# ubisoft/ubisoft-laforge-msmd

Hardware: AMD Instinct MI355X
Metric: FLAME frames/sec on 4s@16kHz clips (whole job; MSMD.forward motion-coefficient frames) (higher is better)
Workload: dtype bf16; 1 GPU; configs[1]: MSMD.forward, batch=32 x 4 s clips per GPU, wav2vec2-base encoder + 8-layer motion decoder, eval-mode, synthetic closed-form weights; batch_per_gpu=32, frames_per_clip=100, parallelism=dp1 (independent clips, no collective), launch=one hipGraph replay per step (the batch sits in the captured input buffers)

## Files before the change

### include/msmd_hip.h

```cpp
#ifndef MSMD_HIP_H
#define MSMD_HIP_H

#include <stdint.h>

#ifdef __cplusplus
extern "C" {
#endif

#define MSMD_F32 0
#define MSMD_BF16 1
#define MSMD_F16 2
#define MSMD_F16X2 3

#define MSMD_ACT_NONE 0
#define MSMD_ACT_GELU 1
#define MSMD_ACT_ELU 2

typedef void* msmd_stream_t;

int msmd_abi_version(void);
#define MSMD_GEMM_VARIANT(v) ((v) << 8)
#define MSMD_GEMM_WRITE_THROUGH (1 << 16)
#define MSMD_GEMM_PAIRED_STORES (1 << 17)
#define MSMD_GEMM_STAGGER (1 << 18)
// ... 42 lines not shown
                       const float* gamma, const float* beta, void* y, int rows, int cols, float eps, int dtype,
                       msmd_stream_t stream);

int msmd_layernorm_f16x2(const float* x, const float* residual, const float* gamma, const float* beta,
                         const float* post_add, float* y, void* y_split, int rows, int cols, float eps, int act,
                         msmd_stream_t stream);

int msmd_split_f16x2(const float* x, void* y, long rows, int cols, long ldx, int cols_out, msmd_stream_t stream);
int msmd_unsplit_f16x2(const void* x, float* y, long rows, int cols, int cols_in, long ldy, msmd_stream_t stream);

int msmd_attention_prefetch(const void* Q, const void* K, const void* V, void* O, int B, int H, int Tq, int Tk,
                            long q_bstride, long q_tstride, long k_bstride, long k_tstride, long v_bstride,
                            long v_tstride, long o_bstride, long o_tstride, float scale, const uint8_t* mask, int dtype,
                            const void* const* prefetch_ptrs, const long* prefetch_bytes, int n_prefetch,
                            msmd_stream_t stream);
int msmd_attention(const void* Q, const void* K, const void* V, void* O, int B, int H, int Tq, int Tk,
                   long q_bstride, long q_tstride, long k_bstride, long k_tstride, long v_bstride,
                   long v_tstride, long o_bstride, long o_tstride, float scale, const uint8_t* mask,
                   int dtype, msmd_stream_t stream);

int msmd_attention_f16x2(const void* Q, const void* K, const void* V, void* O, int B, int H, int Tq, int Tk,
                         long q_bstride, long q_tstride, long k_bstride, long k_tstride, long v_bstride,
                         long v_tstride, long o_bstride, long o_tstride, float scale, const uint8_t* mask,
                         int out_dtype, msmd_stream_t stream);


int msmd_person_query_attention(const void* x, long x_seq_stride, const void* Wq, const float* bq, const void* K,
                                const void* V, long kv_bstride, long kv_tstride, void* out, int N, int H, int Tk, int d,
                                float scale, int dtype, msmd_stream_t stream);
int msmd_person_query_attention_ln(const void* x, long x_seq_stride, const void* Wq, const float* bq,
                                   const float* wq_colsum, float ln_eps, const void* K, const void* V, long kv_bstride,
                                   long kv_tstride, void* out, int N, int H, int Tk, int d, float scale, int dtype,
                                   msmd_stream_t stream);

int msmd_attention_dropout(const void* Q, const void* K, const void* V, void* O, int B, int H, int Tq, int Tk,
                           long q_bstride, long q_tstride, long k_bstride, long k_tstride, long v_bstride,
                           long v_tstride, long o_bstride, long o_tstride, float scale, const uint8_t* mask,
                           float p_drop, const unsigned long* rng_state, unsigned int site, int dtype,
                           msmd_stream_t stream);
int msmd_attention_dropout_prefetch(const void* Q, const void* K, const void* V, void* O, int B, int H, int Tq, int Tk,
                                    long q_bstride, long q_tstride, long k_bstride, long k_tstride, long v_bstride,
                                    long v_tstride, long o_bstride, long o_tstride, float scale, const uint8_t* mask,
                                    float p_drop, const unsigned long* rng_state, unsigned int site, int dtype,
                                    const void* const* prefetch_ptrs, const long* prefetch_bytes, int n_prefetch,
                                    msmd_stream_t stream);

int msmd_dropout(const void* x, const void* residual, void* y, long n, float p, const unsigned long* rng_state,
                 unsigned int site, int dtype, msmd_stream_t stream);

int msmd_attention_bwd(const void* Q, const void* K, const void* V, const void* dO, void* dQ, void* dK, void* dV,
                       int B, int H, int Tq, int Tk, long q_bstride, long q_tstride, long k_bstride,
                       long k_tstride, long v_bstride, long v_tstride, long do_bstride, long do_tstride,
                       long dq_bstride, long dq_tstride, long dk_bstride, long dk_tstride, long dv_bstride,
                       long dv_tstride, float scale, const uint8_t* mask, float p_drop,
                       const unsigned long* rng_state, unsigned int site, msmd_stream_t stream);

int msmd_pad_audio(const float* audio, float* out, int B, int L, int reflect_len, int replicate_len,
                   msmd_stream_t stream);

#define MSMD_CONV0_SPLITS 16
int msmd_conv0_stats(const float* audio, const float* w0, float* stats, float* ws, int B, int L, int reflect_len,
                     int replicate_len, int C, float eps, msmd_stream_t stream);

int msmd_conv0_gn_gelu(const float* audio, const float* w0, const float* stats, const float* gamma,
                       const float* beta, void* out, int B, int L, int reflect_len, int replicate_len,
                       int C, int out_dtype, msmd_stream_t stream);
// ... 148 lines not shown
```

### ubisoft-laforge-msmd_amd/csrc/attention.hip

```cpp
#include "common.h"

struct AttnArgs {
  const void* Q; const void* K; const void* V; void* O;
  int B, H, Tq, Tk;
  long qb, qt, kb, kt, vb, vt, ob, ot;
  float scale;
  const uint8_t* mask;
  float p_drop;
  const unsigned long* rng_state;
  unsigned site;
  const void* pf_ptr[4] = {nullptr, nullptr, nullptr, nullptr};
  long pf_bytes[4] = {0, 0, 0, 0};
};

typedef short s16x4 __attribute__((ext_vector_type(4)));

template <typename T, int NW>
__global__ __launch_bounds__(64 * NW) void attn_kernel(const AttnArgs p) {
  constexpr bool BF = sizeof(T) == 2;
  constexpr int KROW = BF ? 128 : 256;
  constexpr int VROW = BF ? 128 : 272;
  constexpr int NCH = BF ? 8 : 16;
  __shared__ __attribute__((aligned(16))) unsigned char smem[64 * KROW + 64 * VROW + 1024];
  unsigned char* sK = smem;
// ... 193 lines not shown
      }
    } else {
#pragma unroll
      for (int f = 0; f < 4; ++f)
#pragma unroll
        for (int e = 0; e < 4; ++e) {
          const int krow = 16 * f + 4 * fq + e;
#pragma unroll
          for (int d = 0; d < 4; ++d) {
            const float a = *(const float*)(sV + krow * 272 + (16 * d + fr) * 4);
            acc_o[d] = __builtin_amdgcn_mfma_f32_16x16x4f32(a, s[f][e], acc_o[d], 0, 0, 0);
          }
        }
    }
  }

  if (query < p.Tq) {
    const float inv = 1.0f / (l_run * (1.0f - p.p_drop));
    T* Op = (T*)p.O + (long)b * p.ob + (long)query * p.ot + h * 64;
#pragma unroll
    for (int d = 0; d < 4; ++d) {
      float o[4];
#pragma unroll
      for (int e = 0; e < 4; ++e) o[e] = acc_o[d][e] * inv;
      if constexpr (BF)
        *(typename Vec4T<T>::type*)(Op + 16 * d + 4 * fq) = pack4<T>(o[0], o[1], o[2], o[3]);
      else
        *(f32x4*)(Op + 16 * d + 4 * fq) = f32x4{o[0], o[1], o[2], o[3]};
    }
  }
}

constexpr int ATTN_WHOLE_NF = 13;

template <typename T, int NW, int NF = ATTN_WHOLE_NF>
__global__ __launch_bounds__(64 * NW) void attn_whole_kernel(const AttnArgs p) {
  static_assert(sizeof(T) == 2, "16-bit storage modes");
  constexpr int ROWS = 16 * NF, NT = 64 * NW;
  extern __shared__ __attribute__((aligned(16))) unsigned char smem[];
  unsigned char* sK = smem;
  const int tid = threadIdx.x, lane = tid & 63, wid = tid >> 6;
  const int fr = lane & 15, fq = lane >> 4;
  const int b = blockIdx.z, h = blockIdx.y;
  const int query = blockIdx.x * (16 * NW) + wid * 16 + fr;
  const int qrow = query < p.Tq ? query : p.Tq - 1;
  const T* Qp = (const T*)p.Q + (long)b * p.qb + (long)qrow * p.qt + h * 64;
  const T* Kb = (const T*)p.K + (long)b * p.kb + h * 64;
  const T* Vb = (const T*)p.V + (long)b * p.vb + h * 64;
  const int nf = (p.Tk + 15) >> 4;
  const int rows = min(((nf + 1) & ~1) * 16, ROWS);
  unsigned char* sV = smem + rows * 128;

  constexpr int NPF = (ROWS * 8 + NT - 1) / NT;
  u32x4 pk[NPF], pv[NPF];
#pragma unroll
  for (int i = 0; i < NPF; ++i) {
    const int c = tid + i * NT, row = min(c >> 3, p.Tk - 1), ch = c & 7;
    pk[i] = *(const u32x4*)(Kb + (long)row * p.kt + ch * 8);
    pv[i] = *(const u32x4*)(Vb + (long)row * p.vt + ch * 8);
  }
  u32x4 qf[2];
#pragma unroll
  for (int g = 0; g < 2; ++g) qf[g] = *(const u32x4*)(Qp + 32 * g + 8 * fq);
  __builtin_amdgcn_sched_barrier(0);
#pragma unroll
  for (int i = 0; i < NPF; ++i) {
    const int c = tid + i * NT, row = c >> 3, ch = c & 7;
    if (row < rows) {
      const bool live = row < p.Tk;
      *(u32x4*)(sK + row * 128 + ((ch ^ ((row >> 1) & 7)) << 4)) = live ? pk[i] : u32x4{0, 0, 0, 0};
      *(u32x4*)(sV + row * 128 + ((((ch >> 1) ^ ((row >> 1) & 3)) << 5) + ((ch & 1) << 4))) = live ? pv[i] : u32x4{0, 0, 0, 0};
    }
  }
  __syncthreads();
  asm volatile("" ::"v"(qf[0]), "v"(qf[1]));
  if (p.pf_bytes[0] > 0) {
    typedef __attribute__((address_space(3))) void lds_sink_t;
    const unsigned sink_lds = (unsigned)(uintptr_t)(lds_sink_t*)smem + 2 * rows * 128;
    unsigned m0_keep;
    const long stride = (long)gridDim.x * gridDim.y * gridDim.z * NT * 16;
    const long wave0 = ((((long)blockIdx.z * gridDim.y + blockIdx.y) * gridDim.x + blockIdx.x) * NT + (tid & ~63)) * 16;
#pragma unroll
    for (int r = 0; r < 4; ++r) {
      const char* base = (const char*)p.pf_ptr[r];
      const long nb = p.pf_bytes[r] & ~1023L;
      for (long off = wave0; off < nb; off += stride)
        asm volatile("s_mov_b32 %0, m0\n\ts_mov_b32 m0, %2\n\ts_nop 0\n\tglobal_load_lds_dwordx4 %1, off\n\ts_mov_b32 m0, %0"
                     : "=&s"(m0_keep) : "v"(base + off + lane * 16), "s"(sink_lds) : "memory");
    }
  }

  f32x4 s[NF];
#pragma unroll
  for (int f = 0; f < NF; ++f) {
    s[f] = f32x4{0.f, 0.f, 0.f, 0.f};
    if (f >= nf) continue;
    const int row = 16 * f + fr;
#pragma unroll
    for (int g = 0; g < 2; ++g) {
      const u32x4 a = *(const u32x4*)(sK + row * 128 + (((4 * g + fq) ^ ((row >> 1) & 7)) << 4));
      s[f] = mfma16<T>(a, qf[g], s[f]);
    }
  }
  if ((p.Tk & 15) || p.mask) {
    const uint8_t* mrow = p.mask ? p.mask + (long)qrow * p.Tk : nullptr;
#pragma unroll
    for (int f = 0; f < NF; ++f) {
      if (f >= nf || !(p.mask || f == nf - 1)) continue;
      const int k0 = 16 * f + 4 * fq;
      unsigned m4 = 0;
      if (mrow) {
        if (k0 + 4 <= p.Tk) __builtin_memcpy(&m4, mrow + k0, 4);
        else {
#pragma unroll
          for (int e = 0; e < 4; ++e)
            if (k0 + e < p.Tk) m4 |= (unsigned)(mrow[k0 + e] != 0) << (8 * e);
        }
      }
#pragma unroll
      for (int e = 0; e < 4; ++e)
        if (k0 + e >= p.Tk || ((m4 >> (8 * e)) & 0xff)) s[f][e] = -INFINITY;
    }
  }
  const float c = p.scale * 1.4426950408889634f;
  float mx = -INFINITY;
#pragma unroll
  for (int f = 0; f < NF; ++f) {
    if (f >= nf) continue;
#pragma unroll
    for (int e = 0; e < 4; ++e) mx = fmaxf(mx, s[f][e]);
  }
  mx = fmaxf(mx, __shfl_xor(mx, 16, 64));
  mx = fmaxf(mx, __shfl_xor(mx, 32, 64));
  const float mc = (mx == -INFINITY) ? 0.f : mx * c;
  float ps = 0.f;
#pragma unroll
  for (int f = 0; f < NF; ++f) {
    if (f >= nf) continue;
#pragma unroll
    for (int e = 0; e < 4; ++e) {
      const float pe = __builtin_amdgcn_exp2f(fmaf(s[f][e], c, -mc));
      s[f][e] = pe;
      ps += pe;
    }
  }
  ps += __shfl_xor(ps, 16, 64);
  ps += __shfl_xor(ps, 32, 64);
  if (p.p_drop > 0.f) {
    const unsigned thr = dropout_threshold16(p.p_drop);
    const unsigned long rowbase = ((unsigned long)(b * p.H + h) * p.Tq + qrow) * 128ul;
#pragma unroll
    for (int pr = 0; pr < (NF + 1) / 2; ++pr) {
      if (2 * pr >= nf) continue;
      const Philox4 r = dropout_bits(p.rng_state, p.site, rowbase + (unsigned long)(4 * pr + fq));
#pragma unroll
      for (int o = 0; o < 2; ++o) {
        if (2 * pr + o >= NF) continue;
#pragma unroll
        for (int e = 0; e < 4; ++e) s[2 * pr + o][e] = dropout_value16(r, e, o) >= thr ? s[2 * pr + o][e] : 0.f;
      }
    }
  }

  f32x4 acc_o[4];
#pragma unroll
  for (int d = 0; d < 4; ++d) acc_o[d] = f32x4{0.f, 0.f, 0.f, 0.f};
  typedef typename Vec8T<T>::type V8;
  typedef short s16x8 __attribute__((ext_vector_type(8)));
  const int qp = fr >> 2, pp = fr & 3;
#pragma unroll
  for (int pr = 0; pr < (NF + 1) / 2; ++pr) {
    const int f0 = 2 * pr, f1 = 2 * pr + 1;
    if (f0 >= nf) continue;
    const f32x4 s1 = f1 < NF ? s[f1 < NF ? f1 : 0] : f32x4{0.f, 0.f, 0.f, 0.f};
    const V8 pbv = V8{(T)s[f0][0], (T)s[f0][1], (T)s[f0][2], (T)s[f0][3], (T)s1[0], (T)s1[1], (T)s1[2], (T)s1[3]};
    const u32x4 pb = __builtin_bit_cast(u32x4, pbv);
    const int r0 = 16 * f0 + 4 * fq + qp, r1 = f1 < NF ? r0 + 16 : r0;
#pragma unroll
    for (int d = 0; d < 4; ++d) {
      const s16x4 v0 = __builtin_amdgcn_ds_read_tr16_b64_v4i16(
          (s16x4 __attribute__((address_space(3)))*)(sV + r0 * 128 + ((d ^ ((r0 >> 1) & 3)) << 5) + pp * 8));
      const s16x4 v1 = __builtin_amdgcn_ds_read_tr16_b64_v4i16(
          (s16x4 __attribute__((address_space(3)))*)(sV + r1 * 128 + ((d ^ ((r1 >> 1) & 3)) << 5) + pp * 8));
      const s16x8 va = s16x8{v0[0], v0[1], v0[2], v0[3], v1[0], v1[1], v1[2], v1[3]};
      acc_o[d] = mfma16<T>(__builtin_bit_cast(u32x4, va), pb, acc_o[d]);
    }
  }
  if (query < p.Tq) {
    const float inv = 1.0f / (ps * (1.0f - p.p_drop));
    T* Op = (T*)p.O + (long)b * p.ob + (long)query * p.ot + h * 64;
#pragma unroll
    for (int d = 0; d < 4; ++d)
      *(typename Vec4T<T>::type*)(Op + 16 * d + 4 * fq) = pack4<T>(acc_o[d][0] * inv, acc_o[d][1] * inv, acc_o[d][2] * inv, acc_o[d][3] * inv);
  }
  asm volatile("s_waitcnt vmcnt(0)" ::: "memory");
}

__device__ __forceinline__ int vsw(int row) { return ((row & 3) << 2) | ((row >> 2) & 3); }

template <typename TO, int NW>
__global__ __launch_bounds__(64 * NW) void attn_split_kernel(const AttnArgs p) {
  __shared__ __attribute__((aligned(16))) unsigned char smem[2 * 64 * 256];
  unsigned char* sK = smem;
  unsigned char* sV = smem + 64 * 256;
  const int tid = threadIdx.x, lane = tid & 63, wid = tid >> 6;
  const int fr = lane & 15, fq = lane >> 4;
  const int b = blockIdx.z, h = blockIdx.y;
  constexpr int NT = 64 * NW;
  const int query = blockIdx.x * (16 * NW) + wid * 16 + fr;
  const int qrow = query < p.Tq ? query : p.Tq - 1;
  const f16_t* Qp = (const f16_t*)p.Q + 2 * ((long)b * p.qb + (long)qrow * p.qt) + h * 128;
  const f16_t* Kb = (const f16_t*)p.K + 2 * (long)b * p.kb + h * 128;
  const f16_t* Vb = (const f16_t*)p.V + 2 * (long)b * p.vb + h * 128;

  u32x4 qh[2], ql[2];
#pragma unroll
  for (int g = 0; g < 2; ++g) {
    qh[g] = *(const u32x4*)(Qp + 64 * g + 8 * fq);
    ql[g] = *(const u32x4*)(Qp + 64 * g + 32 + 8 * fq);
  }
  f32x4 o0[4], o1[4];
#pragma unroll
  for (int d = 0; d < 4; ++d) o0[d] = o1[d] = f32x4{0.f, 0.f, 0.f, 0.f};
  float m_run = -INFINITY, l_run = 0.f;

  constexpr int NPF = (64 * 16 + NT - 1) / NT;
  u32x4 pk[NPF], pv[NPF];
// ... 220 lines not shown
                        o_bstride, o_tstride, scale, mask, 0.f, nullptr, 0u, dtype, stream);
}

extern "C" int msmd_attention_prefetch(const void* Q, const void* K, const void* V, void* O, int B, int H, int Tq, int Tk,
                                       long q_bstride, long q_tstride, long k_bstride, long k_tstride, long v_bstride,
                                       long v_tstride, long o_bstride, long o_tstride, float scale, const uint8_t* mask,
                                       int dtype, const void* const* prefetch_ptrs, const long* prefetch_bytes,
                                       int n_prefetch, msmd_stream_t stream) {
  return attention_impl(Q, K, V, O, B, H, Tq, Tk, q_bstride, q_tstride, k_bstride, k_tstride, v_bstride, v_tstride,
                        o_bstride, o_tstride, scale, mask, 0.f, nullptr, 0u, dtype, stream, prefetch_ptrs, prefetch_bytes,
                        n_prefetch);
}

extern "C" int msmd_attention_dropout(const void* Q, const void* K, const void* V, void* O, int B, int H, int Tq,
                                      int Tk, long q_bstride, long q_tstride, long k_bstride, long k_tstride,
                                      long v_bstride, long v_tstride, long o_bstride, long o_tstride, float scale,
                                      const uint8_t* mask, float p_drop, const unsigned long* rng_state,
                                      unsigned int site, int dtype, msmd_stream_t stream) {
  return attention_impl(Q, K, V, O, B, H, Tq, Tk, q_bstride, q_tstride, k_bstride, k_tstride, v_bstride, v_tstride,
                        o_bstride, o_tstride, scale, mask, p_drop, rng_state, site, dtype, stream);
}

extern "C" int msmd_attention_dropout_prefetch(const void* Q, const void* K, const void* V, void* O, int B, int H, int Tq,
                                               int Tk, long q_bstride, long q_tstride, long k_bstride, long k_tstride,
                                               long v_bstride, long v_tstride, long o_bstride, long o_tstride, float scale,
                                               const uint8_t* mask, float p_drop, const unsigned long* rng_state,
                                               unsigned int site, int dtype, const void* const* prefetch_ptrs,
                                               const long* prefetch_bytes, int n_prefetch, msmd_stream_t stream) {
  return attention_impl(Q, K, V, O, B, H, Tq, Tk, q_bstride, q_tstride, k_bstride, k_tstride, v_bstride, v_tstride,
                        o_bstride, o_tstride, scale, mask, p_drop, rng_state, site, dtype, stream, prefetch_ptrs,
                        prefetch_bytes, n_prefetch);
}

extern "C" int msmd_attention_f16x2(const void* Q, const void* K, const void* V, void* O, int B, int H, int Tq, int Tk,
                                    long q_bstride, long q_tstride, long k_bstride, long k_tstride, long v_bstride,
                                    long v_tstride, long o_bstride, long o_tstride, float scale, const uint8_t* mask,
                                    int out_dtype, msmd_stream_t stream) {
  if (B <= 0 || H <= 0 || Tq <= 0 || Tk <= 0 || !Q || !K || !V || !O) return 1;
  if (out_dtype != MSMD_F32 && out_dtype != MSMD_F16X2) return 1;
  if (q_tstride % 32 || k_tstride % 32 || v_tstride % 32 || q_bstride % 32 || k_bstride % 32 || v_bstride % 32) return 1;
  if (out_dtype == MSMD_F16X2 ? (o_tstride % 32 || o_bstride % 32) : (o_tstride % 4 || o_bstride % 4)) return 1;
  if (((uintptr_t)Q & 15) || ((uintptr_t)K & 15) || ((uintptr_t)V & 15) || ((uintptr_t)O & 15)) return 1;
  AttnArgs p{Q, K, V, O, B, H, Tq, Tk, q_bstride, q_tstride, k_bstride, k_tstride, v_bstride, v_tstride,
             o_bstride, o_tstride, scale, mask, 0.f, nullptr, 0u};
  const int nw = attn_waves(Tq, H, B);
  dim3 grid((Tq + 16 * nw - 1) / (16 * nw), H, B), block(64 * nw);
  hipStream_t st = (hipStream_t)stream;
#define MSMD_ATTN_S(TO)                                                                                \
  do {                                                                                                 \
    if (nw == 4) hipLaunchKernelGGL((attn_split_kernel<TO, 4>), grid, block, 0, st, p);                \
    else if (nw == 7) hipLaunchKernelGGL((attn_split_kernel<TO, 7>), grid, block, 0, st, p);           \
    else if (nw == 13) hipLaunchKernelGGL((attn_split_kernel<TO, 13>), grid, block, 0, st, p);         \
    else hipLaunchKernelGGL((attn_split_kernel<TO, 16>), grid, block, 0, st, p);                       \
  } while (0)
  if (out_dtype == MSMD_F32) MSMD_ATTN_S(float);
  else MSMD_ATTN_S(f16_t);
#undef MSMD_ATTN_S
  MSMD_RETURN_LAST();
}



template <typename T> __device__ __forceinline__ void load8(const T* p, float (&o)[8]) {
  if constexpr (sizeof(T) == 4) {
    const f32x4 a = *(const f32x4*)p, b = *(const f32x4*)(p + 4);
#pragma unroll
// ... 212 lines not shown
```

### ubisoft-laforge-msmd_amd/model.py

```python
from __future__ import annotations

from types import SimpleNamespace

import torch
import torch.nn as nn

from . import init, ops, shapes, synth
from .utils.model_common import ParamTree, PositionalEncoding, enc_dec_mask, sinusoid_table


def _cd(args) -> torch.dtype:
    name = getattr(args, "compute_dtype", "bf16")
    if name in ("bf16", torch.bfloat16):
        return torch.bfloat16
    if name in ("fp32", "float32", torch.float32):
        return torch.float32
    if name in ("f16x2", "split"):
        return torch.float32
    if name in ("fp16", "float16", "half", torch.float16):
        return torch.float16
    raise ValueError(f"Unknown compute dtype {name}!")


def _is_split(args) -> bool:
# ... 261 lines not shown
        out = []
        for L, kv in zip(P.layers, kv_list):
            N, Tk, _ = kv.shape
            R = torch.zeros(N, Tk + 1, d, device=kv.device, dtype=dtype)
            v = kv[..., d:]
            if P.split:
                v = ops.to_split(kv)[..., d:]
            ops.gemm(v, L.ca_ow, L.ca_ob, None, ops.ACT_NONE, out=R[:, 1:, :], M=Tk, N=d, K=d, lda=2 * d, ldc=d, batch=N,
                     strideA=Tk * 2 * d, strideW=0, strideC=(Tk + 1) * d)
            out.append(R)
        return out

    def trunk(self, feats, tok0, mem, dtype, kv_list=None, row0_add=None, cross_list=None):
        P = self.pack(dtype)
        d, H = self.feature_dim, self.n_heads
        N, Tn, _ = feats.shape
        x = ops.gemm(feats, *P.fp)
        ops.add_pe_token(x, P.pe, tok0, row0_add)
        scale = (d // H) ** -0.5
        if P.split:
            return self._trunk_split(P, x, mem, kv_list, cross_list, scale)
        diag = P.diag and getattr(self, "diag_fast_path", True) and (cross_list is not None or
                                                                     getattr(self, "diag_single_pass", False))
        if diag and cross_list is None:
            if kv_list is None:
                kv_list = self.memory_kv(mem, dtype)
            cross_list = self.memory_cross(kv_list, dtype)
        fold = P.fold and ops.FOLD_LN
        if kv_list is None and not diag:
            kv_list = self.memory_kv(mem, dtype, stacked=True)
        if fold and not diag:
            u = st = ln = None
            for li, L in enumerate(P.layers):
                if li == 0:
                    qkv = ops.gemm(x, L.sa_w, L.sa_b)
                else:
                    qkv = ops.gemm_ln(u, L.f_sa[0], L.f_sa[2], a_stats=st, w_colsum=L.f_sa[1])
                a = ops.attention(qkv[..., :d], qkv[..., d:2 * d], qkv[..., 2 * d:], H, scale,
                                  prefetch=(L.sa_ow, L.f_caq[0], L.ca_ow))
                if li == 0:
                    u1, st1 = ops.gemm_ln(a, L.sa_ow, L.sa_ob, x, stats_out=True)
                else:
                    u1, st1 = ops.gemm_ln(a, L.sa_ow, L.sa_ob, u, r_stats=st, r_gamma=ln[0], r_beta=ln[1], stats_out=True)
                kv = kv_list[li] if kv_list is not None else ops.gemm(mem, L.ca_kvw, L.ca_kvb)
                q = ops.gemm_ln(u1, L.f_caq[0], L.f_caq[2], a_stats=st1, w_colsum=L.f_caq[1])
                nxt = P.layers[li + 1].f_sa[0] if li + 1 < len(P.layers) else P.md0[0]
                c = ops.attention(q, kv[..., :d], kv[..., d:], H, scale, mask=P.mask, prefetch=(L.f_l1[0], L.l2[0], nxt))
                u2, st2 = ops.gemm_ln(c, L.ca_ow, L.ca_ob, u1, r_stats=st1, r_gamma=L.n1[0], r_beta=L.n1[1], stats_out=True)
                f = ops.gemm_ln(u2, L.f_l1[0], L.f_l1[2], act=ops.ACT_GELU, a_stats=st2, w_colsum=L.f_l1[1])
                u, st = ops.gemm_ln(f, L.l2[0], L.l2[1], u2, r_stats=st2, r_gamma=L.n2[0], r_beta=L.n2[1], stats_out=True)
                ln = L.n3
            x = ops.layernorm(u, *ln)
        u = st = ln = None
        n_layers = len(P.layers)
        for li, L in enumerate(P.layers if not (fold and not diag) else ()):
            if u is None:
                qkv = ops.gemm(x, L.sa_w, L.sa_b)
            else:
                qkv = ops.gemm_ln(u, L.f_sa[0], L.f_sa[2], a_stats=st, w_colsum=L.f_sa[1])
            nxt = None
            if li + 1 < len(P.layers):
                nxt = P.layers[li + 1].f_sa[0] if (fold and diag) else P.layers[li + 1].sa_w
            a = ops.attention(qkv[..., :d], qkv[..., d:2 * d], qkv[..., 2 * d:], H, scale,
                              prefetch=None if P.split else (L.sa_ow, L.l1[0], L.l2[0], nxt))
            fused_pq = getattr(self, "fused_person_query", True)
            fold_n1 = fold and diag and fused_pq
            u1 = ops.gemm(a, L.sa_ow, L.sa_ob, residual=x) if u is None else \
                ops.gemm_ln(a, L.sa_ow, L.sa_ob, u, r_stats=st, r_gamma=ln[0], r_beta=ln[1])
            if not fold_n1:
                x = ops.layernorm(u1, *L.n1)
            kv = kv_list[li] if kv_list is not None else ops.gemm(mem, L.ca_kvw, L.ca_kvb)
            last = li + 1 == n_layers
# ... 381 lines not shown
```

### ubisoft-laforge-msmd_amd/ops.py

```python
from __future__ import annotations

import ctypes
import os

import torch

from . import _lib

F32, BF16, F16, F16X2 = 0, 1, 2, 3
SPLIT = "f16x2"


class Split:
    __slots__ = ("t", "below_32")
    dtype = SPLIT
    is_cuda = True

    def __init__(self, t, below_32=False):
        if t.dtype != torch.float16 or t.shape[-1] % 64 or t.stride(-1) != 1:
            raise TypeError("Split wraps an fp16 tensor whose last dim is 2 x (a multiple of 32)")
        self.t = t
        self.below_32 = below_32

    @property
# ... 119 lines not shown
        if t is not None and not t.is_cuda:
            raise RuntimeError("msmd_amd ops need tensors on the MI355X (cuda) device; there is no CPU path")


GEMM_AUTOTUNE = os.environ.get("MSMD_GEMM_AUTOTUNE", "0") == "1"
_TUNE_MIN_FLOP = 1.0e9
_TUNE_CANDIDATES = (17, 13, 9, 12)
_TUNED = {}
GEMM_WRITE_THROUGH, GEMM_PAIRED_STORES, GEMM_STAGGER = 1 << 16, 1 << 17, 1 << 18
GEMM_ONE_TILE_PER_WORKGROUP = 1 << 19
GEMM_NO_256_TILE = 1 << 20
GEMM_W_BELOW_32 = 1 << 21
GEMM_LN_FLAGS = 0
GEMM_LN_ROUTER = None
GEMM_LN_ALL_IN_ONE = False


class capture_guard:

    def __enter__(self):
        import gc
        gc.collect()
        self.was = gc.isenabled()
        gc.disable()
        return self

    def __exit__(self, *exc):
        import gc
        if self.was:
            gc.enable()
        return False
PREFETCH_WEIGHTS = os.environ.get("MSMD_PREFETCH", "1") != "0"
FOLD_LN = os.environ.get("MSMD_FOLD_LN", "1") != "0"
GEMM_ROUTER = None
_GEMM_DEFAULT = {"variant": 0, "flags": GEMM_PAIRED_STORES, "split_variant": 0}
if os.environ.get("MSMD_GEMM_ONE_TILE", "0") == "1":
    _GEMM_DEFAULT["flags"] |= GEMM_ONE_TILE_PER_WORKGROUP
    GEMM_LN_FLAGS = GEMM_ONE_TILE_PER_WORKGROUP


if os.environ.get("MSMD_GEMM_NO_256", "0") == "1":
    _GEMM_DEFAULT["flags"] |= GEMM_NO_256_TILE
    GEMM_LN_FLAGS |= GEMM_NO_256_TILE


class gemm_defaults:

    def __init__(self, variant=None, flags=None, split_variant=None):
        self.new = {k: v for k, v in (("variant", variant), ("flags", flags), ("split_variant", split_variant))
                    if v is not None}

    def __enter__(self):
        self.old = dict(_GEMM_DEFAULT)
        _GEMM_DEFAULT.update(self.new)
        return self

    def __exit__(self, *exc):
        _GEMM_DEFAULT.clear()
        _GEMM_DEFAULT.update(self.old)
        return False


def _autotune_gemm(lib, args, key, out, residual):
    if torch.cuda.is_current_stream_capturing() or (residual is not None and residual.data_ptr() == out.data_ptr()):
        return 0
    act = args[16]
# ... 285 lines not shown
    if out is None:
        out = torch.empty(B, Tq, d, device=q.device, dtype=q.dtype)
    m = None
    if mask is not None:
        assert mask.dtype in (torch.bool, torch.uint8) and mask.shape == (Tq, Tk) and mask.is_contiguous()
        m = mask
    if p_drop > 0.0 and prefetch and PREFETCH_WEIGHTS:
        ptrs, nbytes, n = _prefetch_ranges(prefetch)
        _lib.check(lib.msmd_attention_dropout_prefetch(_p(q), _p(k), _p(v), _p(out), B, n_heads, Tq, Tk, q.stride(0),
                                                       q.stride(1), k.stride(0), k.stride(1), v.stride(0), v.stride(1),
                                                       out.stride(0), out.stride(1), float(scale), _p(m), float(p_drop),
                                                       _p(rng_state), int(site), _dt(q), ptrs, nbytes, n, _stream()),
                   "msmd_attention_dropout_prefetch")
        return out
    if p_drop > 0.0:
        _lib.check(lib.msmd_attention_dropout(_p(q), _p(k), _p(v), _p(out), B, n_heads, Tq, Tk, q.stride(0),
                                              q.stride(1), k.stride(0), k.stride(1), v.stride(0), v.stride(1),
                                              out.stride(0), out.stride(1), float(scale), _p(m), float(p_drop),
                                              _p(rng_state), int(site), _dt(q), _stream()), "msmd_attention_dropout")
        return out
    if prefetch and PREFETCH_WEIGHTS:
        ptrs, nbytes, n = _prefetch_ranges(prefetch)
        _lib.check(lib.msmd_attention_prefetch(_p(q), _p(k), _p(v), _p(out), B, n_heads, Tq, Tk, q.stride(0), q.stride(1),
                                               k.stride(0), k.stride(1), v.stride(0), v.stride(1), out.stride(0),
                                               out.stride(1), float(scale), _p(m), _dt(q), ptrs, nbytes, n,
                                               _stream()), "msmd_attention_prefetch")
        return out
    _lib.check(lib.msmd_attention(_p(q), _p(k), _p(v), _p(out), B, n_heads, Tq, Tk, q.stride(0), q.stride(1),
                                  k.stride(0), k.stride(1), v.stride(0), v.stride(1), out.stride(0), out.stride(1),
                                  float(scale), _p(m), _dt(q), _stream()), "msmd_attention")
    return out


def attention_bwd(q, k, v, do, dq, dk, dv, n_heads, scale, mask=None, p_drop=0.0, rng_state=None, site=0):
    _need_cuda(q, k, v, do, dq, dk, dv)
    lib = _lib.load()
    B, Tq, d = q.shape
    Tk = k.shape[1]
    for t in (q, k, v, do, dq, dk, dv):
        if t.dtype != torch.bfloat16 or t.stride(-1) != 1:
            raise TypeError("attention_bwd takes bf16 tensors with a contiguous last dim")
    m = None
    if mask is not None:
        assert mask.dtype in (torch.bool, torch.uint8) and mask.shape == (Tq, Tk) and mask.is_contiguous()
        m = mask
    _lib.check(lib.msmd_attention_bwd(_p(q), _p(k), _p(v), _p(do), _p(dq), _p(dk), _p(dv), B, n_heads, Tq, Tk,
                                      q.stride(0), q.stride(1), k.stride(0), k.stride(1), v.stride(0), v.stride(1),
                                      do.stride(0), do.stride(1), dq.stride(0), dq.stride(1), dk.stride(0),
                                      dk.stride(1), dv.stride(0), dv.stride(1), float(scale), _p(m), float(p_drop),
                                      _p(rng_state), int(site), _stream()),
               "msmd_attention_bwd")


def dynamic_threshold_(res, L, ratio, dt_min, dt_max):
    _need_cuda(res)
    if res.dtype != torch.float32 or not res.is_contiguous():
        raise TypeError("dynamic_threshold_ takes a contiguous fp32 tensor")
    N, T_all, C = res.shape
    _lib.check(_lib.load().msmd_dynamic_threshold(_p(res), N, T_all, L, C, float(ratio), float(dt_min), float(dt_max),
                                                  _stream()), "msmd_dynamic_threshold")
    return res


def pad_audio(audio, reflect_len, replicate_len):
    lib = _lib.load()
    B, L = audio.shape
# ... 470 lines not shown
```

Baseline: 832,100 frames/s.

## Fuse QKV projection (with folded LayerNorm) into the whole-sequence attention kernel

Adds a qkv_attn_kernel in which each (batch, head) workgroup computes its own Q/K/V slice of the QKV projection from the input rows, streaming weights through a double-buffered LDS ring. It applies the folded LayerNorm correction and bias, writes K/V/Q directly into the swizzled LDS layout, and then runs the existing whole-sequence attention body. The decoder self-attention path uses it when T <= 112. This removes the separate QKV GEMM launch and the round trip of the QKV tensor through global memory. In exchange, grid parallelism is limited to B*H workgroups, each doing a serial K-loop over the full hidden size, so the projection may run on fewer compute units than a tiled GEMM would.

Result: no change. 838,600 frames/s (median of 6 runs) (+0.8%).

```diff
diff --git a/include/msmd_hip.h b/include/msmd_hip.h
--- a/include/msmd_hip.h
+++ b/include/msmd_hip.h
@@ -98,6 +98,11 @@
                                    const float* wq_colsum, float ln_eps, const void* K, const void* V, long kv_bstride,
                                    long kv_tstride, void* out, int N, int H, int Tk, int d, float scale, int dtype,
                                    msmd_stream_t stream);
+
+int msmd_qkv_attention(const void* X, long x_bstride, long x_tstride, const void* Wqkv, const float* bias,
+                       const float* w_colsum, const float* a_stats, int a_nt, float ln_eps, void* O, long o_bstride,
+                       long o_tstride, int B, int H, int T, float scale, int dtype, const void* const* prefetch_ptrs,
+                       const long* prefetch_bytes, int n_prefetch, msmd_stream_t stream);
 
 int msmd_attention_dropout(const void* Q, const void* K, const void* V, void* O, int B, int H, int Tq, int Tk,
                            long q_bstride, long q_tstride, long k_bstride, long k_tstride, long v_bstride,
diff --git a/ubisoft-laforge-msmd_amd/csrc/attention.hip b/ubisoft-laforge-msmd_amd/csrc/attention.hip
--- a/ubisoft-laforge-msmd_amd/csrc/attention.hip
+++ b/ubisoft-laforge-msmd_amd/csrc/attention.hip
@@ -249,6 +249,131 @@
 }
 
 constexpr int ATTN_WHOLE_NF = 13;
+
+template <int NT>
+__device__ __forceinline__ void attn_prefetch_ranges(const AttnArgs& p, unsigned sink_lds) {
+  const int tid = threadIdx.x, lane = tid & 63;
+  unsigned m0_keep;
+  const long stride = (long)gridDim.x * gridDim.y * gridDim.z * NT * 16;
+  const long wave0 = ((((long)blockIdx.z * gridDim.y + blockIdx.y) * gridDim.x + blockIdx.x) * NT + (tid & ~63)) * 16;
+#pragma unroll
+  for (int r = 0; r < 4; ++r) {
+    const char* base = (const char*)p.pf_ptr[r];
+    const long nb = p.pf_bytes[r] & ~1023L;
+    for (long off = wave0; off < nb; off += stride)
+      asm volatile("s_mov_b32 %0, m0\n\ts_mov_b32 m0, %2\n\ts_nop 0\n\tglobal_load_lds_dwordx4 %1, off\n\ts_mov_b32 m0, %0"
+                   : "=&s"(m0_keep) : "v"(base + off + lane * 16), "s"(sink_lds) : "memory");
+  }
+}
+
+template <typename T, int NF>
+__device__ __forceinline__ void attn_whole_body(const AttnArgs& p, const unsigned char* sK, const unsigned char* sV,
+                                                const u32x4 (&qf)[2], int nf, int b, int h, int query, int qrow) {
+  const int lane = threadIdx.x & 63, fr = lane & 15, fq = lane >> 4;
+  f32x4 s[NF];
+#pragma unroll
+  for (int f = 0; f < NF; ++f) {
+    s[f] = f32x4{0.f, 0.f, 0.f, 0.f};
+    if (f >= nf) continue;
+    const int row = 16 * f + fr;
+#pragma unroll
+    for (int g = 0; g < 2; ++g) {
+      const u32x4 a = *(const u32x4*)(sK + row * 128 + (((4 * g + fq) ^ ((row >> 1) & 7)) << 4));
+      s[f] = mfma16<T>(a, qf[g], s[f]);
+    }
+  }
+  if ((p.Tk & 15) || p.mask) {
+    const uint8_t* mrow = p.mask ? p.mask + (long)qrow * p.Tk : nullptr;
+#pragma unroll
+    for (int f = 0; f < NF; ++f) {
+      if (f >= nf || !(p.mask || f == nf - 1)) continue;
+      const int k0 = 16 * f + 4 * fq;
+      unsigned m4 = 0;
+      if (mrow) {
+        if (k0 + 4 <= p.Tk) __builtin_memcpy(&m4, mrow + k0, 4);
+        else {
+#pragma unroll
+          for (int e = 0; e < 4; ++e)
+            if (k0 + e < p.Tk) m4 |= (unsigned)(mrow[k0 + e] != 0) << (8 * e);
+        }
+      }
+#pragma unroll
+      for (int e = 0; e < 4; ++e)
+        if (k0 + e >= p.Tk || ((m4 >> (8 * e)) & 0xff)) s[f][e] = -INFINITY;
+    }
+  }
+  const float c = p.scale * 1.4426950408889634f;
+  float mx = -INFINITY;
+#pragma unroll
+  for (int f = 0; f < NF; ++f) {
+    if (f >= nf) continue;
+#pragma unroll
+    for (int e = 0; e < 4; ++e) mx = fmaxf(mx, s[f][e]);
+  }
+  mx = fmaxf(mx, __shfl_xor(mx, 16, 64));
+  mx = fmaxf(mx, __shfl_xor(mx, 32, 64));
+  const float mc = (mx == -INFINITY) ? 0.f : mx * c;
+  float ps = 0.f;
+#pragma unroll
+  for (int f = 0; f < NF; ++f) {
+    if (f >= nf) continue;
+#pragma unroll
+    for (int e = 0; e < 4; ++e) {
+      const float pe = __builtin_amdgcn_exp2f(fmaf(s[f][e], c, -mc));
+      s[f][e] = pe;
+      ps += pe;
+    }
+  }
+  ps += __shfl_xor(ps, 16, 64);
+  ps += __shfl_xor(ps, 32, 64);
+  if (p.p_drop > 0.f) {
+    const unsigned thr = dropout_threshold16(p.p_drop);
+    const unsigned long rowbase = ((unsigned long)(b * p.H + h) * p.Tq + qrow) * 128ul;
+#pragma unroll
+    for (int pr = 0; pr < (NF + 1) / 2; ++pr) {
+      if (2 * pr >= nf) continue;
+      const Philox4 r = dropout_bits(p.rng_state, p.site, rowbase + (unsigned long)(4 * pr + fq));
+#pragma unroll
+      for (int o = 0; o < 2; ++o) {
+        if (2 * pr + o >= NF) continue;
+#pragma unroll
+        for (int e = 0; e < 4; ++e) s[2 * pr + o][e] = dropout_value16(r, e, o) >= thr ? s[2 * pr + o][e] : 0.f;
+      }
+    }
+  }
+
+  f32x4 acc_o[4];
+#pragma unroll
+  for (int d = 0; d < 4; ++d) acc_o[d] = f32x4{0.f, 0.f, 0.f, 0.f};
+  typedef typename Vec8T<T>::type V8;
+  typedef short s16x8 __attribute__((ext_vector_type(8)));
+  const int qp = fr >> 2, pp = fr & 3;
+#pragma unroll
+  for (int pr = 0; pr < (NF + 1) / 2; ++pr) {
+    const int f0 = 2 * pr, f1 = 2 * pr + 1;
+    if (f0 >= nf) continue;
+    const f32x4 s1 = f1 < NF ? s[f1 < NF ? f1 : 0] : f32x4{0.f, 0.f, 0.f, 0.f};
+    const V8 pbv = V8{(T)s[f0][0], (T)s[f0][1], (T)s[f0][2], (T)s[f0][3], (T)s1[0], (T)s1[1], (T)s1[2], (T)s1[3]};
+    const u32x4 pb = __builtin_bit_cast(u32x4, pbv);
+    const int r0 = 16 * f0 + 4 * fq + qp, r1 = f1 < NF ? r0 + 16 : r0;
+#pragma unroll
+    for (int d = 0; d < 4; ++d) {
+      const s16x4 v0 = __builtin_amdgcn_ds_read_tr16_b64_v4i16(
+          (s16x4 __attribute__((address_space(3)))*)(sV + r0 * 128 + ((d ^ ((r0 >> 1) & 3)) << 5) + pp * 8));
+      const s16x4 v1 = __builtin_amdgcn_ds_read_tr16_b64_v4i16(
+          (s16x4 __attribute__((address_space(3)))*)(sV + r1 * 128 + ((d ^ ((r1 >> 1) & 3)) << 5) + pp * 8));
+      const s16x8 va = s16x8{v0[0], v0[1], v0[2], v0[3], v1[0], v1[1], v1[2], v1[3]};
+      acc_o[d] = mfma16<T>(__builtin_bit_cast(u32x4, va), pb, acc_o[d]);
+    }
+  }
+  if (query < p.Tq) {
+    const float inv = 1.0f / (ps * (1.0f - p.p_drop));
+    T* Op = (T*)p.O + (long)b * p.ob + (long)query * p.ot + h * 64;
+#pragma unroll
+    for (int d = 0; d < 4; ++d)
+      *(typename Vec4T<T>::type*)(Op + 16 * d + 4 * fq) = pack4<T>(acc_o[d][0] * inv, acc_o[d][1] * inv, acc_o[d][2] * inv, acc_o[d][3] * inv);
+  }
+}
 
 template <typename T, int NW, int NF = ATTN_WHOLE_NF>
 __global__ __launch_bounds__(64 * NW) void attn_whole_kernel(const AttnArgs p) {
@@ -293,123 +418,143 @@
   asm volatile("" ::"v"(qf[0]), "v"(qf[1]));
   if (p.pf_bytes[0] > 0) {
     typedef __attribute__((address_space(3))) void lds_sink_t;
-    const unsigned sink_lds = (unsigned)(uintptr_t)(lds_sink_t*)smem + 2 * rows * 128;
+    attn_prefetch_ranges<NT>(p, (unsigned)(uintptr_t)(lds_sink_t*)smem + 2 * rows * 128);
+  }
+
+  attn_whole_body<T, NF>(p, sK, sV, qf, nf, b, h, query, qrow);
+  asm volatile("s_waitcnt vmcnt(0)" ::: "memory");
+}
+
+struct QkvAttnArgs {
+  AttnArgs a;
+  const void* X; long xb, xt;
+  const void* W; const float* bias;
+  const float* colsum;
+  const float* stats; int nt, M;
+  float eps;
+  int d;
+};
+
+template <typename T, int NW, bool LNA, int NF = ATTN_WHOLE_NF>
+__global__ __launch_bounds__(64 * NW) void qkv_attn_kernel(const QkvAttnArgs q) {
+  static_assert(sizeof(T) == 2 && 16 * NW <= 16 * NF, "16-bit storage; one workgroup holds every row");
+  constexpr int ROWS = 16 * NF, NT = 64 * NW, STAGE = 192 * 128, LPW = (24 + NW - 1) / NW;
+  extern __shared__ __attribute__((aligned(16))) unsigned char smem[];
+  typedef __attribute__((address_space(3))) void lds_t;
+  const AttnArgs& p = q.a;
+  const int tid = threadIdx.x, lane = tid & 63, wid = tid >> 6;
+  const int fr = lane & 15, fq = lane >> 4;
+  const int h = blockIdx.x % p.H, b = blockIdx.x / p.H;
+  const int d = q.d, nk = d / 64;
+  const int m = 16 * wid + fr, mrow = min(m, p.Tq - 1);
+  const T* xr = (const T*)q.X + (long)b * q.xb + (long)mrow * q.xt + 8 * fq;
+
+  const T* src[LPW];
+#pragma unroll
+  for (int i = 0; i < LPW; ++i) {
+    const int j = min(i * NW + wid, 23), id = j * 64 + lane, row = id >> 3;
+    const int c = (id & 7) ^ ((row >> 1) & 7);
+    src[i] = (const T*)q.W + (long)((row >> 6) * d + 64 * h + (row & 63)) * d + c * 8;
+  }
+  const unsigned ring = (unsigned)(uintptr_t)(lds_t*)smem;
+  const int wv = __builtin_amdgcn_readfirstlane(wid);
+  auto issue = [&](int kt, int st) {
     unsigned m0_keep;
-    const long stride = (long)gridDim.x * gridDim.y * gridDim.z * NT * 16;
-    const long wave0 = ((((long)blockIdx.z * gridDim.y + blockIdx.y) * gridDim.x + blockIdx.x) * NT + (tid & ~63)) * 16;
+#pragma unroll
+    for (int i = 0; i < LPW; ++i)
+      if (i * NW + wv < 24)
+        asm volatile("s_mov_b32 %0, m0\n\ts_mov_b32 m0, %2\n\ts_nop 0\n\tglobal_load_lds_dwordx4 %1, off\n\ts_mov_b32 m0, %0"
+                     : "=&s"(m0_keep)
+                     : "v"(src[i] + kt * 64), "s"(ring + st * STAGE + (i * NW + wv) * 1024) : "memory");
+  };
+
+  f32x4 raw[4];
+  if constexpr (LNA) {
+    const f32x2* sp = (const f32x2*)q.stats + (long)b * p.Tq + mrow;
 #pragma unroll
     for (int r = 0; r < 4; ++r) {
-      const char* base = (const char*)p.pf_ptr[r];
-      const long nb = p.pf_bytes[r] & ~1023L;
-      for (long off = wave0; off < nb; off += stride)
-        asm volatile("s_mov_b32 %0, m0\n\ts_mov_b32 m0, %2\n\ts_nop 0\n\tglobal_load_lds_dwordx4 %1, off\n\ts_mov_b32 m0, %0"
-                     : "=&s"(m0_keep) : "v"(base + off + lane * 16), "s"(sink_lds) : "memory");
-    }
-  }
-
-  f32x4 s[NF];
-#pragma unroll
-  for (int f = 0; f < NF; ++f) {
-    s[f] = f32x4{0.f, 0.f, 0.f, 0.f};
-    if (f >= nf) continue;
-    const int row = 16 * f + fr;
-#pragma unroll
-    for (int g = 0; g < 2; ++g) {
-      const u32x4 a = *(const u32x4*)(sK + row * 128 + (((4 * g + fq) ^ ((row >> 1) & 7)) << 4));
-      s[f] = mfma16<T>(a, qf[g], s[f]);
-    }
-  }
-  if ((p.Tk & 15) || p.mask) {
-    const uint8_t* mrow = p.mask ? p.mask + (long)qrow * p.Tk : nullptr;
-#pragma unroll
-    for (int f = 0; f < NF; ++f) {
-      if (f >= nf || !(p.mask || f == nf - 1)) continue;
-      const int k0 = 16 * f + 4 * fq;
-      unsigned m4 = 0;
-      if (mrow) {
-        if (k0 + 4 <= p.Tk) __builtin_memcpy(&m4, mrow + k0, 4);
-        else {
-#pragma unroll
-          for (int e = 0; e < 4; ++e)
-            if (k0 + e < p.Tk) m4 |= (unsigned)(mrow[k0 + e] != 0) << (8 * e);
-        }
-      }
-#pragma unroll
-      for (int e = 0; e < 4; ++e)
-        if (k0 + e >= p.Tk || ((m4 >> (8 * e)) & 0xff)) s[f][e] = -INFINITY;
-    }
-  }
-  const float c = p.scale * 1.4426950408889634f;
-  float mx = -INFINITY;
-#pragma unroll
-  for (int f = 0; f < NF; ++f) {
-    if (f >= nf) continue;
-#pragma unroll
-    for (int e = 0; e < 4; ++e) mx = fmaxf(mx, s[f][e]);
-  }
-  mx = fmaxf(mx, __shfl_xor(mx, 16, 64));
-  mx = fmaxf(mx, __shfl_xor(mx, 32, 64));
-  const float mc = (mx == -INFINITY) ? 0.f : mx * c;
-  float ps = 0.f;
-#pragma unroll
-  for (int f = 0; f < NF; ++f) {
-    if (f >= nf) continue;
+      const f32x2 w = fq + 4 * r < q.nt ? sp[(long)(fq + 4 * r) * q.M] : f32x2{0.f, 0.f};
+      raw[r] = f32x4{w[0], w[1], 0.f, 0.f};
+    }
+  }
+  f32x4 acc[12];
+#pragma unroll
+  for (int i = 0; i < 12; ++i) acc[i] = f32x4{0.f, 0.f, 0.f, 0.f};
+  u32x4 xf[2], xn[2];
+#pragma unroll
+  for (int g = 0; g < 2; ++g) xf[g] = *(const u32x4*)(xr + 32 * g);
+  issue(0, 0);
+  for (int kt = 0; kt < nk; ++kt) {
+    asm volatile("s_waitcnt vmcnt(0)" ::: "memory");
+    __builtin_amdgcn_s_barrier();
+    if (kt + 1 < nk) {
+#pragma unroll
+      for (int g = 0; g < 2; ++g) xn[g] = *(const u32x4*)(xr + (kt + 1) * 64 + 32 * g);
+      issue(kt + 1, (kt + 1) & 1);
+    }
+    const unsigned char* sw = smem + (kt & 1) * STAGE;
+#pragma unroll
+    for (int g = 0; g < 2; ++g)
+#pragma unroll
+      for (int i = 0; i < 12; ++i) {
+        const int row = 16 * i + fr;
+        const u32x4 fw = *(const u32x4*)(sw + row * 128 + (((4 * g + fq) ^ ((row >> 1) & 7)) << 4));
+        acc[i] = mfma16<T>(fw, xf[g], acc[i]);
+      }
+    if (kt + 1 < nk) { xf[0] = xn[0]; xf[1] = xn[1]; }
+  }
+
+  float mu = 0.f, rs = 1.f;
+  if constexpr (LNA) {
+    float S = (raw[0][0] + raw[1][0]) + (raw[2][0] + raw[3][0]);
+    float Q = (raw[0][1] + raw[1][1]) + (raw[2][1] + raw[3][1]);
+    S += __shfl_xor(S, 16, 64); S += __shfl_xor(S, 32, 64);
+    Q += __shfl_xor(Q, 16, 64); Q += __shfl_xor(Q, 32, 64);
+    const float inv_cols = 1.0f / (float)d;
+    mu = S * inv_cols;
+    rs = rsqrtf(fmaxf(Q * inv_cols - mu * mu, 0.f) + q.eps);
+  }
+  const int nf = (p.Tk + 15) >> 4;
+  const int rows = min(((nf + 1) & ~1) * 16, ROWS);
+  unsigned char* sK = smem;
+  unsigned char* sV = smem + rows * 128;
+  unsigned char* sQ = smem + 2 * ROWS * 128 + wid * 2048;
+  __syncthreads();
+  typedef typename Vec4T<T>::type V4;
+#pragma unroll
+  for (int i = 0; i < 12; ++i) {
+    const int col = (i >> 2) * d + 64 * h + (i & 3) * 16 + 4 * fq;
+    const f32x4 bv = *(const f32x4*)(q.bias + col);
+    f32x4 cx = f32x4{0.f, 0.f, 0.f, 0.f};
+    if constexpr (LNA) cx = *(const f32x4*)(q.colsum + col);
+    float v[4];
 #pragma unroll
     for (int e = 0; e < 4; ++e) {
-      const float pe = __builtin_amdgcn_exp2f(fmaf(s[f][e], c, -mc));
-      s[f][e] = pe;
-      ps += pe;
-    }
-  }
-  ps += __shfl_xor(ps, 16, 64);
-  ps += __shfl_xor(ps, 32, 64);
-  if (p.p_drop > 0.f) {
-    const unsigned thr = dropout_threshold16(p.p_drop);
-    const unsigned long rowbase = ((unsigned long)(b * p.H + h) * p.Tq + qrow) * 128ul;
-#pragma unroll
-    for (int pr = 0; pr < (NF + 1) / 2; ++pr) {
-      if (2 * pr >= nf) continue;
-      const Philox4 r = dropout_bits(p.rng_state, p.site, rowbase + (unsigned long)(4 * pr + fq));
-#pragma unroll
-      for (int o = 0; o < 2; ++o) {
-        if (2 * pr + o >= NF) continue;
-#pragma unroll
-        for (int e = 0; e < 4; ++e) s[2 * pr + o][e] = dropout_value16(r, e, o) >= thr ? s[2 * pr + o][e] : 0.f;
-      }
-    }
-  }
-
-  f32x4 acc_o[4];
-#pragma unroll
-  for (int d = 0; d < 4; ++d) acc_o[d] = f32x4{0.f, 0.f, 0.f, 0.f};
-  typedef typename Vec8T<T>::type V8;
-  typedef short s16x8 __attribute__((ext_vector_type(8)));
-  const int qp = fr >> 2, pp = fr & 3;
-#pragma unroll
-  for (int pr = 0; pr < (NF + 1) / 2; ++pr) {
-    const int f0 = 2 * pr, f1 = 2 * pr + 1;
-    if (f0 >= nf) continue;
-    const f32x4 s1 = f1 < NF ? s[f1 < NF ? f1 : 0] : f32x4{0.f, 0.f, 0.f, 0.f};
-    const V8 pbv = V8{(T)s[f0][0], (T)s[f0][1], (T)s[f0][2], (T)s[f0][3], (T)s1[0], (T)s1[1], (T)s1[2], (T)s1[3]};
-    const u32x4 pb = __builtin_bit_cast(u32x4, pbv);
-    const int r0 = 16 * f0 + 4 * fq + qp, r1 = f1 < NF ? r0 + 16 : r0;
-#pragma unroll
-    for (int d = 0; d < 4; ++d) {
-      const s16x4 v0 = __builtin_amdgcn_ds_read_tr16_b64_v4i16(
-          (s16x4 __attribute__((address_space(3)))*)(sV + r0 * 128 + ((d ^ ((r0 >> 1) & 3)) << 5) + pp * 8));
-      const s16x4 v1 = __builtin_amdgcn_ds_read_tr16_b64_v4i16(
-          (s16x4 __attribute__((address_space(3)))*)(sV + r1 * 128 + ((d ^ ((r1 >> 1) & 3)) << 5) + pp * 8));
-      const s16x8 va = s16x8{v0[0], v0[1], v0[2], v0[3], v1[0], v1[1], v1[2], v1[3]};
-      acc_o[d] = mfma16<T>(__builtin_bit_cast(u32x4, va), pb, acc_o[d]);
-    }
-  }
-  if (query < p.Tq) {
-    const float inv = 1.0f / (ps * (1.0f - p.p_drop));
-    T* Op = (T*)p.O + (long)b * p.ob + (long)query * p.ot + h * 64;
-#pragma unroll
-    for (int d = 0; d < 4; ++d)
-      *(typename Vec4T<T>::type*)(Op + 16 * d + 4 * fq) = pack4<T>(acc_o[d][0] * inv, acc_o[d][1] * inv, acc_o[d][2] * inv, acc_o[d][3] * inv);
-  }
+      float x = acc[i][e];
+      if constexpr (LNA) x = rs * (x - mu * cx[e]);
+      v[e] = x + bv[e];
+    }
+    const V4 o = pack4<T>(v[0], v[1], v[2], v[3]);
+    const int ch = 2 * (i & 3) + (fq >> 1), sub = (fq & 1) * 8;
+    if (i < 4) {
+      *(V4*)(sQ + fr * 128 + ((ch ^ ((fr >> 1) & 7)) << 4) + sub) = o;
+    } else if (m < rows) {
+      const V4 w = m < p.Tk ? o : V4{};
+      if (i < 8) *(V4*)(sK + m * 128 + ((ch ^ ((m >> 1) & 7)) << 4) + sub) = w;
+      else *(V4*)(sV + m * 128 + ((((ch >> 1) ^ ((m >> 1) & 3)) << 5) + ((ch & 1) << 4)) + sub) = w;
+    }
+  }
+  for (int c = tid; c < (rows - 16 * NW) * 8; c += NT) {
+    const int row = 16 * NW + (c >> 3);
+    *(u32x4*)(sK + row * 128 + (c & 7) * 16) = u32x4{0, 0, 0, 0};
+    *(u32x4*)(sV + row * 128 + (c & 7) * 16) = u32x4{0, 0, 0, 0};
+  }
+  __syncthreads();
+  u32x4 qf[2];
+#pragma unroll
+  for (int g = 0; g < 2; ++g) qf[g] = *(const u32x4*)(sQ + fr * 128 + (((4 * g + fq) ^ ((fr >> 1) & 7)) << 4));
+  if (p.pf_bytes[0] > 0) attn_prefetch_ranges<NT>(p, ring + 2 * ROWS * 128 + NW * 2048);
+  attn_whole_body<T, NF>(p, sK, sV, qf, nf, b, h, m, mrow);
   asm volatile("s_waitcnt vmcnt(0)" ::: "memory");
 }
 
@@ -696,6 +841,49 @@
                         prefetch_bytes, n_prefetch);
 }
 
+extern "C" int msmd_qkv_attention(const void* X, long x_bstride, long x_tstride, const void* Wqkv, const float* bias,
+                                  const float* w_colsum, const float* a_stats, int a_nt, float ln_eps, void* O,
+                                  long o_bstride, long o_tstride, int B, int H, int T, float scale, int dtype,
+                                  const void* const* prefetch_ptrs, const long* prefetch_bytes, int n_prefetch,
+                                  msmd_stream_t stream) {
+  const int d = 64 * H;
+  if (B <= 0 || H <= 0 || T <= 0 || T > 16 * ATTN_WHOLE_NF || !X || !Wqkv || !bias || !O || !(scale > 0.f)) return 1;
+  if (dtype != MSMD_BF16 && dtype != MSMD_F16) return 1;
+  if (x_tstride % 8 || x_bstride % 8 || o_tstride % 4 || o_bstride % 4 || x_tstride < d || o_tstride < d) return 1;
+  if (((uintptr_t)X & 15) || ((uintptr_t)Wqkv & 15) || ((uintptr_t)bias & 15) || ((uintptr_t)O & 15)) return 1;
+  const bool lna = a_stats != nullptr;
+  if (lna && (!w_colsum || ((uintptr_t)w_colsum & 15) || a_nt * 64 != d || a_nt > 16)) return 1;
+  if (n_prefetch < 0 || n_prefetch > 4 || (n_prefetch > 0 && (!prefetch_ptrs || !prefetch_bytes))) return 1;
+  QkvAttnArgs q{};
+  q.a = AttnArgs{nullptr, nullptr, nullptr, O, B, H, T, T, 0, 0, 0, 0, 0, 0, o_bstride, o_tstride, scale, nullptr, 0.f,
+                 nullptr, 0u};
+  for (int i = 0, j = 0; i < n_prefetch; ++i)
+    if (prefetch_ptrs[i] && prefetch_bytes[i] >= 16 && ((uintptr_t)prefetch_ptrs[i] & 15) == 0) {
+      q.a.pf_ptr[j] = prefetch_ptrs[i]; q.a.pf_bytes[j] = prefetch_bytes[i]; ++j;
+    }
+  q.X = X; q.xb = x_bstride; q.xt = x_tstride; q.W = Wqkv; q.bias = bias;
+  q.colsum = w_colsum; q.stats = a_stats; q.nt = a_nt; q.M = B * T; q.eps = ln_eps; q.d = d;
+  hipStream_t st = (hipStream_t)stream;
+#define MSMD_QKV_W(TT, NWV, LN)                                                                                      \
+  do {                                                                                                               \
+    constexpr int lds_ = 2 * 16 * ATTN_WHOLE_NF * 128 + NWV * 2048 + 1024;                                           \
+    static bool attr_ = false;                                                                                       \
+    auto k_ = qkv_attn_kernel<TT, NWV, LN>;                                                                          \
+    if (!attr_) { (void)hipFuncSetAttribute((const void*)k_, hipFuncAttributeMaxDynamicSharedMemorySize, lds_); attr_ = true; } \
+    hipLaunchKernelGGL(k_, dim3(B * H), dim3(64 * NWV), lds_, st, q);                                                \
+  } while (0)
+#define MSMD_QKV_T(TT)                                                                                               \
+  do {                                                                                                               \
+    if (T <= 112) { if (lna) MSMD_QKV_W(TT, 7, true); else MSMD_QKV_W(TT, 7, false); }                              \
+    else { if (lna) MSMD_QKV_W(TT, 13, true); else MSMD_QKV_W(TT, 13, false); }                                      \
+  } while (0)
+  if (dtype == MSMD_BF16) MSMD_QKV_T(bf16_t);
+  else MSMD_QKV_T(f16_t);
+#undef MSMD_QKV_T
+#undef MSMD_QKV_W
+  MSMD_RETURN_LAST();
+}
+
 extern "C" int msmd_attention_f16x2(const void* Q, const void* K, const void* V, void* O, int B, int H, int Tq, int Tk,
                                     long q_bstride, long q_tstride, long k_bstride, long k_tstride, long v_bstride,
                                     long v_tstride, long o_bstride, long o_tstride, float scale, const uint8_t* mask,
diff --git a/ubisoft-laforge-msmd_amd/model.py b/ubisoft-laforge-msmd_amd/model.py
--- a/ubisoft-laforge-msmd_amd/model.py
+++ b/ubisoft-laforge-msmd_amd/model.py
@@ -317,12 +317,18 @@
         if fold and not diag:
             u = st = ln = None
             for li, L in enumerate(P.layers):
-                if li == 0:
-                    qkv = ops.gemm(x, L.sa_w, L.sa_b)
+                pf = (L.sa_ow, L.f_caq[0], L.ca_ow)
+                if ops.qkv_attention_routes(x, H):
+                    if li == 0:
+                        a = ops.qkv_attention(x, L.sa_w, L.sa_b, H, scale, prefetch=pf)
+                    else:
+                        a = ops.qkv_attention(u, L.f_sa[0], L.f_sa[2], H, scale, a_stats=st, w_colsum=L.f_sa[1], prefetch=pf)
                 else:
-                    qkv = ops.gemm_ln(u, L.f_sa[0], L.f_sa[2], a_stats=st, w_colsum=L.f_sa[1])
-                a = ops.attention(qkv[..., :d], qkv[..., d:2 * d], qkv[..., 2 * d:], H, scale,
-                                  prefetch=(L.sa_ow, L.f_caq[0], L.ca_ow))
+                    if li == 0:
+                        qkv = ops.gemm(x, L.sa_w, L.sa_b)
+                    else:
+                        qkv = ops.gemm_ln(u, L.f_sa[0], L.f_sa[2], a_stats=st, w_colsum=L.f_sa[1])
+                    a = ops.attention(qkv[..., :d], qkv[..., d:2 * d], qkv[..., 2 * d:], H, scale, prefetch=pf)
                 if li == 0:
                     u1, st1 = ops.gemm_ln(a, L.sa_ow, L.sa_ob, x, stats_out=True)
                 else:
diff --git a/ubisoft-laforge-msmd_amd/ops.py b/ubisoft-laforge-msmd_amd/ops.py
--- a/ubisoft-laforge-msmd_amd/ops.py
+++ b/ubisoft-laforge-msmd_amd/ops.py
@@ -175,6 +175,7 @@
         return False
 PREFETCH_WEIGHTS = os.environ.get("MSMD_PREFETCH", "1") != "0"
 FOLD_LN = os.environ.get("MSMD_FOLD_LN", "1") != "0"
+FUSED_QKV_ATTN = os.environ.get("MSMD_FUSED_QKV_ATTN", "1") != "0"
 GEMM_ROUTER = None
 _GEMM_DEFAULT = {"variant": 0, "flags": GEMM_PAIRED_STORES, "split_variant": 0}
 if os.environ.get("MSMD_GEMM_ONE_TILE", "0") == "1":
@@ -526,6 +527,31 @@
     return out
 
 
+def qkv_attention_routes(x, n_heads, p_drop=0.0):
+    return (FUSED_QKV_ATTN and not isinstance(x, Split) and x.dtype in (torch.bfloat16, torch.float16) and x.dim() == 3
+            and 1 <= x.shape[1] <= 112 and x.shape[2] == 64 * n_heads and x.shape[2] <= 1024 and x.stride(2) == 1
+            and not p_drop > 0.0)
+
+
+def qkv_attention(x, w, bias, n_heads, scale, *, a_stats=None, w_colsum=None, eps=1e-5, prefetch=None, out=None):
+    _need_cuda(x, w, bias)
+    B, T, d = x.shape
+    if w.shape != (3 * d, d) or not w.is_contiguous() or w.dtype != x.dtype or bias is None or bias.dtype != torch.float32:
+        raise ValueError("qkv_attention: w must be a contiguous (3d, d) weight of x's dtype, bias fp32 (3d,)")
+    nt = 0
+    if a_stats is not None:
+        if w_colsum is None or a_stats.dim() != 3 or a_stats.shape[0] * 64 != d or a_stats.shape[1] != B * T:
+            raise ValueError("qkv_attention: a_stats must be (d / 64, B*T, 2) with w_colsum")
+        nt = a_stats.shape[0]
+    if out is None:
+        out = torch.empty(B, T, d, device=x.device, dtype=x.dtype)
+    ptrs, nbytes, n = _prefetch_ranges(prefetch) if (prefetch and PREFETCH_WEIGHTS) else (None, None, 0)
+    _lib.check(_lib.load().msmd_qkv_attention(_p(x), x.stride(0), x.stride(1), _p(w), _p(bias), _p(w_colsum), _p(a_stats),
+                                              nt, float(eps), _p(out), out.stride(0), out.stride(1), B, n_heads, T,
+                                              float(scale), _dt(x), ptrs, nbytes, n, _stream()), "msmd_qkv_attention")
+    return out
+
+
 def attention_bwd(q, k, v, do, dq, dk, dv, n_heads, scale, mask=None, p_drop=0.0, rng_state=None, site=0):
     _need_cuda(q, k, v, do, dq, dk, dv)
     lib = _lib.load()
```
